# Avokadoen/zig_vulkan

Measured on AMD Instinct MI355X. Metric: Mrays/s at 1920x1080 on 512^3 brickmap (8^3 bricks, primary + shadow, 1 spp); achieved % of HBM roofline, higher is better.
Workload: dtype f32

## Files before the change

zig_vulkan_amd/csrc/vrt_trace_kernels.h:

```cpp
#pragma once
#include <hip/hip_runtime.h>
#include "vrt_internal.h"
#include "vrt_kernels.h"
#include "vrt_math.h"

namespace vrt {

constexpr uint32_t MAT_LAMBERTIAN = 0, MAT_METAL = 1, MAT_DIELECTRIC = 2, MAT_NONE = 3;

struct Ray {
    f3 origin, direction;
    float internal_reflection;
    uint32_t ignore_type_material;
};

struct Hit {
    f3 point, normal;
    float t;
    uint32_t index;
};

template <bool COUNT>
struct Cnt {
    uint32_t rays = 0, status_loads = 0, bricks_entered = 0, voxel_steps = 0, hits = 0, grid_steps = 0;
// ... 714 lines not shown
}

constexpr float kBoxMissEps = 1.0f / 64.0f;
constexpr float kBoxMissReach = 2048.0f;
VRT_DI bool box_miss(const f3 &origin, const f3 &inv_dir, const int (&bounds)[6], const f3 &g_min, float g_scale) {
    float reach = 0.0f;
    auto slab = [&](int k, float o, float inv, float g, float &near, float &far) {
        const float lo = ((float)(-bounds[k]) - (1.0f + kBoxMissEps)) * g_scale + g;
        const float hi = ((float)bounds[k + 3] + (2.0f + kBoxMissEps)) * g_scale + g;
        const float a0 = lo - o, a1 = hi - o;
        const float t0 = a0 * inv, t1 = a1 * inv;
        near = __builtin_fminf(t0, t1);
        far = __builtin_fmaxf(t0, t1);
        reach = __builtin_fmaxf(reach, __builtin_fmaxf(__builtin_fmaxf(__builtin_fabsf(a0), __builtin_fabsf(a1)), __builtin_fabsf(o)));
    };
    float nx, fx, ny, fy, nz, fz;
    slab(0, origin.x, inv_dir.x, g_min.x, nx, fx);
    slab(1, origin.y, inv_dir.y, g_min.y, ny, fy);
    slab(2, origin.z, inv_dir.z, g_min.z, nz, fz);
    const float tn = __builtin_fmaxf(__builtin_fmaxf(__builtin_fmaxf(nx, ny), nz), 0.0f);
    const float tf = __builtin_fminf(__builtin_fminf(fx, fy), fz);
    const float inv_max = __builtin_fmaxf(__builtin_fmaxf(__builtin_fabsf(inv_dir.x), __builtin_fabsf(inv_dir.y)), __builtin_fabsf(inv_dir.z));
    return tf < tn && reach <= kBoxMissReach * g_scale && inv_max < __builtin_inff();
}

struct BrickConsts {
    BrickArgs a;
    uint32_t occupancy_words;
    uint32_t start_is_slot;
    uint32_t scale_pow2;
    float inv_voxel_scale;
};
template <typename T>
VRT_DI T opaque_uniform(T v) {
    asm volatile("" : "+s"(v));
    return v;
}
template <typename T>
VRT_DI const __attribute__((address_space(1))) T *global_ptr(const T *ptr) {
    return (const __attribute__((address_space(1))) T *)ptr;
}
VRT_DI uint32_t scalar_load_u32(const uint32_t *ptr) {
    uint32_t v;
    asm volatile("s_load_dword %0, %1, 0x0\n\ts_waitcnt lgkmcnt(0)" : "=s"(v) : "s"(ptr));
    return v;
}
typedef __attribute__((ext_vector_type(8))) uint32_t u32x8;
typedef __attribute__((ext_vector_type(16))) uint32_t u32x16;
typedef __attribute__((ext_vector_type(2))) uint32_t u32x2;
VRT_DI unsigned long long kernarg_address() { return (unsigned long long)__builtin_amdgcn_kernarg_segment_ptr(); }
struct DerivedPtrs {
    const int *cell_bounds;
    const uint32_t *start_is_slot;
    uint32_t skip_to_box;
};
VRT_DI TileArgs kernarg_tile_args(DerivedPtrs &dp) {
    u32x16 v;
    u32x2 b, f;
    asm volatile("s_load_dwordx16 %0, %4, %5\n\ts_load_dwordx2 %1, %4, %6\n\ts_load_dwordx2 %2, %4, %7\n\ts_load_dword %3, %4, %8\n\ts_waitcnt lgkmcnt(0)"
                 : "=&s"(v), "=&s"(b), "=&s"(f), "=&s"(dp.skip_to_box)
                 : "s"(kernarg_address()), "n"(offsetof(TraceParams, tile_args)), "n"(offsetof(TraceParams, grid_extra) + offsetof(GridExtra, cell_bounds)),
                   "n"(offsetof(TraceParams, grid_extra) + offsetof(GridExtra, start_is_slot)), "n"(offsetof(TraceParams, grid_extra) + offsetof(GridExtra, skip_to_box)));
    dp.cell_bounds = (const int *)__builtin_bit_cast(unsigned long long, b);
    dp.start_is_slot = (const uint32_t *)__builtin_bit_cast(unsigned long long, f);
    return __builtin_bit_cast(TileArgs, v);
}

struct DerivedWords {
    int bounds[6];
    uint32_t start_is_slot;
};
struct EarlyBox {
    DerivedWords dw;
    float g_min[3], g_scale;
    bool test;
};
VRT_DI vrt_camera_device kernarg_camera_box(uint32_t frame, const DerivedPtrs &dp, EarlyBox &eb) {
    struct Parts { u32x16 a; u32x8 b; } v;
    u32x4 lo, gm;
    u32x2 hi;
    uint32_t flag, sc;
    const unsigned long long ka = kernarg_address();
    const unsigned long long at = ka + offsetof(TraceParams, pcs) + (unsigned long long)frame * sizeof(PushConstants);
    const unsigned long long b = dp.cell_bounds ? (unsigned long long)dp.cell_bounds : ka, f = dp.start_is_slot ? (unsigned long long)dp.start_is_slot : ka;
    asm volatile("s_load_dwordx16 %0, %7, 0x0\n\ts_load_dwordx8 %1, %7, 0x40\n\ts_load_dwordx4 %2, %8, 0x0\n\ts_load_dwordx2 %3, %8, 0x10\n\t"
                 "s_load_dword %4, %9, 0x0\n\ts_load_dwordx4 %5, %10, %11\n\ts_load_dword %6, %10, %12\n\ts_waitcnt lgkmcnt(0)"
                 : "=&s"(v.a), "=&s"(v.b), "=&s"(lo), "=&s"(hi), "=&s"(flag), "=&s"(gm), "=&s"(sc)
                 : "s"(at), "s"(b), "s"(f), "s"(ka), "n"(offsetof(TraceParams, grid) + offsetof(vrt_grid_state, min_point_base_t)),
                   "n"(offsetof(TraceParams, grid) + offsetof(vrt_grid_state, max_point_scale) + 12));
    eb.dw = DerivedWords{{(int)lo.x, (int)lo.y, (int)lo.z, (int)lo.w, (int)hi.x, (int)hi.y}, dp.start_is_slot ? flag : 0u};
    const uint32_t gx = gm.x, gy = gm.y, gz = gm.z;
    eb.g_min[0] = __builtin_bit_cast(float, gx), eb.g_min[1] = __builtin_bit_cast(float, gy), eb.g_min[2] = __builtin_bit_cast(float, gz);
    eb.g_scale = __builtin_bit_cast(float, sc);
    eb.test = dp.cell_bounds != nullptr && dp.skip_to_box != 0u;
    struct Padded { vrt_camera_device cam; uint32_t pad[8]; };
    static_assert(sizeof(Parts) == sizeof(Padded) && offsetof(Parts, b) == 64, "x16 | x8, padded to the alignment of the first");
    return __builtin_bit_cast(Padded, v).cam;
}
VRT_DI vrt_sun_device kernarg_sun(uint32_t frame) {
    u32x8 v;
    const unsigned long long at = kernarg_address() + offsetof(TraceParams, pcs) + (unsigned long long)frame * sizeof(PushConstants) + offsetof(PushConstants, sun);
    asm volatile("s_load_dwordx8 %0, %1, 0x0\n\ts_waitcnt lgkmcnt(0)" : "=&s"(v) : "s"(at));
    return __builtin_bit_cast(vrt_sun_device, v);
}
struct GridArgs {
    vrt_grid_state grid;
    uint32_t scale_pow2;
    float inv_grid_scale, inv_voxel_scale;
    uint32_t skip_to_box;
    const int *cell_bounds;
    uint32_t status_cells, status_words;
    const uint32_t *start_is_slot;
    uint32_t occupancy_words, count_box;
};
static_assert(sizeof(GridArgs) == sizeof(vrt_grid_state) + sizeof(GridExtra) && offsetof(GridArgs, cell_bounds) - 64 == offsetof(GridExtra, cell_bounds) &&
                  offsetof(GridArgs, start_is_slot) - 64 == offsetof(GridExtra, start_is_slot) && offsetof(GridArgs, count_box) - 64 == offsetof(GridExtra, count_box),
              "GridArgs = vrt_grid_state + GridExtra, field for field");
VRT_DI GridArgs kernarg_grid_args() {
    struct Parts { u32x16 grid; u32x8 a; u32x4 b; } v;
    asm volatile("s_load_dwordx16 %0, %3, 0x0\n\ts_load_dwordx8 %1, %3, %4\n\ts_load_dwordx4 %2, %3, %5\n\ts_waitcnt lgkmcnt(0)"
                 : "=&s"(v.grid), "=&s"(v.a), "=&s"(v.b)
                 : "s"(kernarg_address()), "n"(offsetof(TraceParams, grid_extra)), "n"(offsetof(TraceParams, grid_extra) + 32));
    static_assert(sizeof(Parts) == sizeof(GridArgs) + 16 && offsetof(Parts, a) == 64 && offsetof(Parts, b) == 96, "x16 | x8 | x4, padded to the alignment of the first");
    struct Padded { GridArgs g; uint32_t pad[4]; };
    return __builtin_bit_cast(Padded, v).g;
}
VRT_DI DerivedWords scalar_derived_words(const GridArgs &ga) {
    u32x4 lo;
    u32x2 hi;
    uint32_t flag;
    const unsigned long long ka = kernarg_address();
    const unsigned long long b = ga.cell_bounds ? (unsigned long long)ga.cell_bounds : ka, f = ga.start_is_slot ? (unsigned long long)ga.start_is_slot : ka;
    asm volatile("s_load_dwordx4 %0, %3, 0x0\n\ts_load_dwordx2 %1, %3, 0x10\n\ts_load_dword %2, %4, 0x0\n\ts_waitcnt lgkmcnt(0)"
                 : "=&s"(lo), "=&s"(hi), "=&s"(flag)
                 : "s"(b), "s"(f));
    return DerivedWords{{(int)lo.x, (int)lo.y, (int)lo.z, (int)lo.w, (int)hi.x, (int)hi.y}, ga.start_is_slot ? flag : 0u};
}
VRT_DI BrickConsts kernarg_brick_consts(const GridArgs &ga, uint32_t start_is_slot) {
    u32x16 v;
    asm volatile("s_load_dwordx16 %0, %1, %2\n\ts_waitcnt lgkmcnt(0)" : "=&s"(v) : "s"(kernarg_address()), "n"(offsetof(TraceParams, brick_args)));
    return BrickConsts{__builtin_bit_cast(BrickArgs, v), ga.occupancy_words, start_is_slot, ga.scale_pow2, ga.inv_voxel_scale};
}
VRT_DI int steps_left_fresh(int step, int pos, int dim, int zero_budget) {
    unsigned long long gt, lt;
    asm volatile("v_cmp_lt_i32_e64 %0, 0, %1" : "=s"(gt) : "v"(step));
    asm volatile("v_cmp_gt_i32_e64 %0, 0, %1" : "=s"(lt) : "v"(step));
    return __builtin_amdgcn_inverse_ballot_w64(gt) ? (int)((uint32_t)(dim - 1) - (uint32_t)pos) : (__builtin_amdgcn_inverse_ballot_w64(lt) ? pos : zero_budget);
}

template <int B, bool EAGER = true, bool BY_CELL = false, bool VOXEL = false, bool REJECT = false, bool CONSTS = false>
VRT_DI bool brick_walk_gfx950(const TraceParams &p, const BrickConsts &bc, const Ray &r, const RaySetup &s, float g_scale, uint32_t brick_index, f3 brick_min,
                              Hit &hit, int axis_in, int &hit_axis, uint32_t cell = 0u, uint32_t *hit_voxel = nullptr, uint32_t box = 0u) {
    constexpr bool kConsts = CONSTS;
    static_assert(!(CONSTS && BY_CELL), "the by-cell copy is the bounce kernel's");
    const float brick_voxel_scale = 1.0f / (float)B;
    const float voxel_scale = g_scale * brick_voxel_scale;
    const bool pow2 = kConsts ? opaque_uniform(bc.scale_pow2) != 0u : p.scale_pow2 != 0u;
    const f3 fposition = pow2 ? (ray_at(r, hit.t) - brick_min) * (kConsts ? bc.inv_voxel_scale : p.inv_voxel_scale) : (ray_at(r, hit.t) - brick_min) / splat3(voxel_scale);
    Walk w;
    w.side_dist = initial_side_dist(mk3((float)s.sx, (float)s.sy, (float)s.sz), fposition, s.ray_delta());
    const int px = f2i_clamp(__builtin_floorf(fposition.x));
    const int py = f2i_clamp(__builtin_floorf(fposition.y));
    const int pz = f2i_clamp(__builtin_floorf(fposition.z));
    constexpr int kZeroBudget = 3 * B + 8;
    w.rx = kConsts ? steps_left_fresh(s.sx, px, B, kZeroBudget) : steps_left(s.sx, px, B, kZeroBudget);
    w.ry = kConsts ? steps_left_fresh(s.sy, py, B, kZeroBudget) : steps_left(s.sy, py, B, kZeroBudget);
    w.rz = kConsts ? steps_left_fresh(s.sz, pz, B, kZeroBudget) : steps_left(s.sz, pz, B, kZeroBudget);
    w.t_value = 0;
    const float local_t_max = s.grid_t_max - hit.t;
    const bool by_cell = BY_CELL && p.cell_occupancy_lockstep != 0u;
    const uint32_t base = (by_cell ? cell : brick_index) * (uint32_t)(B * B * B);
    uint32_t bit_index = base + ((uint32_t)px + (uint32_t)B * ((uint32_t)pz + (uint32_t)B * (uint32_t)py));
    const uint32_t stride_x = (uint32_t)s.sx, stride_y = (uint32_t)(s.sy * (B * B)), stride_z = (uint32_t)(s.sz * B);
    bool more = more_init(px, py, pz, B) && (0.0f <= local_t_max);
    if constexpr (REJECT) {
        more = more && !brick_reject<B>(fposition, s.inv_dir, box);
        if (__builtin_amdgcn_ballot_w64(more) == 0ull) return false;
    }

    BrickArgs plain;
    if constexpr (!kConsts) plain.brick_occupancy = p.brick_occupancy, plain.brick_start_index = p.brick_start_index, plain.material_index = p.material_index, plain.materials = p.materials;
    const BrickArgs &a = kConsts ? bc.a : plain;
    const uint8_t *const occupancy = by_cell ? p.cell_occupancy : a.brick_occupancy;
    const unsigned long long occ_addr = (unsigned long long)occupancy;
    u32x4 rsrc;
    rsrc.x = (uint32_t)occ_addr;
    rsrc.y = (uint32_t)(occ_addr >> 32) | (4u << 16);
    rsrc.z = by_cell ? p.status_cells * (uint32_t)(B * B * B / 32) : (kConsts ? bc.occupancy_words : p.occupancy_words);
    rsrc.w = 0x00020000u;
    uint32_t word = global_ptr(reinterpret_cast<const uint32_t *>(occupancy))[more ? (bit_index >> 5) : 0u];
    uint32_t brick_material_index = 0u;
    bool start_is_slot;
    if constexpr (kConsts) start_is_slot = opaque_uniform(bc.start_is_slot) != 0u;
    else start_is_slot = p.start_is_slot != nullptr && __builtin_amdgcn_readfirstlane((int)*p.start_is_slot) != 0;
    if constexpr (EAGER) brick_material_index = start_is_slot ? brick_index * (uint32_t)(B * B * B) : (global_ptr(a.brick_start_index)[brick_index] & 0x7FFFFFFFu);
    GridWalkRegs g;
    g.alive = __builtin_amdgcn_ballot_w64(more);
    g.out_x = 0ull;
    g.out_y = 0ull;
    g.t_out = 0.0f;
    bool first = true;
    bool found = false;
    while (g.alive != 0ull) {
        uint32_t solid_bit;
        VRT_PROF_BEGIN(tp2);
        voxel_walk_gfx950(w, s.inv_dir, bit_index, solid_bit, stride_x, stride_y, stride_z, word, rsrc, g, voxel_scale, local_t_max);
        VRT_PROF_END(2, tp2);
        if (g.occ == 0ull) break;
        if (__builtin_amdgcn_inverse_ballot_w64(g.occ)) {
            VRT_PROF_BEGIN(tp4);
            const uint32_t voxel_index = solid_bit - base;
            if constexpr (!EAGER) brick_material_index = start_is_slot ? brick_index * (uint32_t)(B * B * B) : (global_ptr(a.brick_start_index)[brick_index] & 0x7FFFFFFFu);
            const uint32_t mi = global_ptr(a.material_index)[brick_material_index + voxel_index];
            const auto *m = global_ptr(kConsts ? opaque_uniform(a.materials) : a.materials) + mi;
            const uint32_t mtype = m->type;
            const float mdata = m->type_data;
            const bool ignore_brick = (mtype == r.ignore_type_material) && (r.internal_reflection == mdata);
            if (!ignore_brick) {
                const int a = (first && g.stub == 0u)
                                  ? axis_in
                                  : (__builtin_amdgcn_inverse_ballot_w64(g.in_x) ? 0 : (__builtin_amdgcn_inverse_ballot_w64(g.in_y) ? 1 : 2));
                hit.index = mi;
                const float t_offset = voxel_scale * 0.05f;
                hit.t += g.t_in * voxel_scale - t_offset;
                hit_axis = a;
                if constexpr (VOXEL) *hit_voxel = voxel_index;
                found = true;
            }
            VRT_PROF_END(4, tp4);
        }
        asm("s_andn2_b64 %0, %0, %1" : "+s"(g.alive) : "s"(__builtin_amdgcn_ballot_w64(found)) : "scc");
        first = false;
    }
    return found;
}

#ifndef VRT_BRICK_LOAD_AUX
#define VRT_BRICK_LOAD_AUX 0
#endif
VRT_DI void stage_brick_lds(const TraceParams &p, uint32_t occ_slot, bool by_cell, uint32_t wave_lds) {
    const uint32_t *src = reinterpret_cast<const uint32_t *>(by_cell ? p.cell_occupancy : p.brick_occupancy) + (size_t)occ_slot * 16u;
    typedef __attribute__((address_space(3))) void lds_void;
    typedef const __attribute__((address_space(1))) void glb_void;
    lds_void *dst = reinterpret_cast<lds_void *>((size_t)__builtin_amdgcn_readfirstlane(wave_lds));
#pragma unroll
    for (int c = 0; c < 4; c++)
        __builtin_amdgcn_global_load_lds((glb_void *)(src + 4 * c), (lds_void *)((__attribute__((address_space(3))) char *)dst + 1024 * c), 16, 0, VRT_BRICK_LOAD_AUX);
}
constexpr uint32_t kDeferredHit = 0x80000000u;
template <int B, bool LDS = false, bool PRESTAGED = false, bool DEFER = false>
VRT_DI bool brick_walk_park_gfx950(const TraceParams &p, const Ray &r, const RaySetup &s, float g_scale, uint32_t occ_slot, uint32_t cell, bool by_cell,
                                   bool start_is_slot, f3 brick_min, Hit &hit, int axis_in, int &hit_axis, uint32_t wave_lds = 0u) {
    static_assert(!LDS || B == 8, "the LDS layout is written for 64-byte bricks");
    const float brick_voxel_scale = 1.0f / (float)B;
    const float voxel_scale = g_scale * brick_voxel_scale;
    const f3 fposition = p.scale_pow2 ? (ray_at(r, hit.t) - brick_min) * p.inv_voxel_scale : (ray_at(r, hit.t) - brick_min) / splat3(voxel_scale);
    Walk w;
    w.side_dist = initial_side_dist(mk3((float)s.sx, (float)s.sy, (float)s.sz), fposition, s.ray_delta());
    const int px = f2i_clamp(__builtin_floorf(fposition.x));
    const int py = f2i_clamp(__builtin_floorf(fposition.y));
    const int pz = f2i_clamp(__builtin_floorf(fposition.z));
    constexpr int kZeroBudget = 3 * B + 8;
    w.rx = steps_left(s.sx, px, B, kZeroBudget);
    w.ry = steps_left(s.sy, py, B, kZeroBudget);
    w.rz = steps_left(s.sz, pz, B, kZeroBudget);
    w.t_value = 0;
    const float local_t_max = s.grid_t_max - hit.t;
    const uint32_t base = LDS ? 0u : occ_slot * (uint32_t)(B * B * B);
    uint32_t bit_index = base + ((uint32_t)px + (uint32_t)B * ((uint32_t)pz + (uint32_t)B * (uint32_t)py));
    const uint32_t stride_x = (uint32_t)s.sx, stride_y = (uint32_t)(s.sy * (B * B)), stride_z = (uint32_t)(s.sz * B);
    const bool more = more_init(px, py, pz, B) && (0.0f <= local_t_max);

    const uint8_t *const occupancy = by_cell ? p.cell_occupancy : p.brick_occupancy;
    const unsigned long long occ_addr = (unsigned long long)occupancy;
    u32x4 rsrc;
    rsrc.x = (uint32_t)occ_addr;
    rsrc.y = (uint32_t)(occ_addr >> 32) | (4u << 16);
    rsrc.z = by_cell ? p.status_cells * (uint32_t)(B * B * B / 32) : p.occupancy_words;
// ... 118 lines not shown
}
#undef VRT_SKIP_MERGE_STEP
VRT_DI float &comp3(f3 &v, int i) { return i == 0 ? v.x : (i == 1 ? v.y : v.z); }
VRT_DI float comp3(const f3 &v, int i) { return i == 0 ? v.x : (i == 1 ? v.y : v.z); }
template <int A>
VRT_DI void skip_axis(Walk &w, const RaySetup &s, int need, float t, uint32_t &index, uint32_t stride_x, uint32_t stride_y, uint32_t stride_z, bool &more,
                      int &in_axis, float &t_in) {
    constexpr int B1 = (A + 1) % 3, B2 = (A + 2) % 3;
    int *const r[3] = {&w.rx, &w.ry, &w.rz};
    const uint32_t stride[3] = {stride_x, stride_y, stride_z};
    const float t_strict = next_below(t);
    const int n1 = skip_merge_gfx950(comp3(w.side_dist, B1), comp3(s.inv_dir, B1), *r[B1], B1 > A ? t : t_strict);
    const int n2 = skip_merge_gfx950(comp3(w.side_dist, B2), comp3(s.inv_dir, B2), *r[B2], B2 > A ? t : t_strict);
    comp3(w.side_dist, A) = t + comp3(s.ray_delta(), A);
    *r[A] -= need;
    *r[B1] -= n1;
    *r[B2] -= n2;
    index += (uint32_t)need * stride[A] + (uint32_t)n1 * stride[B1] + (uint32_t)n2 * stride[B2];
    more = (*r[A] | *r[B1] | *r[B2]) >= 0;
    in_axis = A;
    t_in = t;
}
template <int A>
VRT_DI void skip_round(Walk &w, const RaySetup &s, int span, uint32_t &index, uint32_t stride_x, uint32_t stride_y, uint32_t stride_z, bool &more,
                       int &in_axis, float &t_in, bool &skipped) {
    const int step_a = A == 0 ? s.sx : (A == 1 ? s.sy : s.sz);
    const int r_a = A == 0 ? w.rx : (A == 1 ? w.ry : w.rz);
    const int need = step_a != 0 ? r_a - span : 0;
    const bool want = more && need > 0;
    if (__builtin_amdgcn_ballot_w64(want) == 0ull) return;
    if (want) {
        float t = comp3(w.side_dist, A);
        skip_add_gfx950(t, comp3(s.inv_dir, A), need - 1);
        skip_axis<A>(w, s, need, t, index, stride_x, stride_y, stride_z, more, in_axis, t_in);
        skipped = true;
    }
}
VRT_DI bool skip_to_box(Walk &w, const RaySetup &s, int span_x, int span_y, int span_z, uint32_t &index, uint32_t stride_x, uint32_t stride_y,
                        uint32_t stride_z, bool &more, int &in_axis, float &t_in) {
    bool skipped = false;
    skip_round<0>(w, s, span_x, index, stride_x, stride_y, stride_z, more, in_axis, t_in, skipped);
    skip_round<1>(w, s, span_y, index, stride_x, stride_y, stride_z, more, in_axis, t_in, skipped);
    skip_round<2>(w, s, span_z, index, stride_x, stride_y, stride_z, more, in_axis, t_in, skipped);
    return skipped;
}

#ifdef VRT_DEV_VARIANTS
#define VRT_DEV_SECTION 6
#include "vrt_trace_kernels_dev.h"
#undef VRT_DEV_SECTION
#endif
VRT_DI f3 opaque_uniform3(const float (&v)[3]) { return mk3(opaque_uniform(v[0]), opaque_uniform(v[1]), opaque_uniform(v[2])); }

template <int B, bool COUNT, int MODE, bool BATCH = false, bool SCALAR_ENTRY = false, bool VOXEL = false, bool REJECT = false, bool KARGS = false>
VRT_DI bool grid_hit(const TraceParams &p, const uint32_t *lds_filter, const Ray &r, Hit &hit, Cnt<COUNT> &c, int *voxel = nullptr,
                     const DerivedWords *early = nullptr, bool sits_out = false) {
    static_assert(!VOXEL || ((MODE == kStatusLinearAlways || MODE == kStatusLinearLds || MODE == kStatusBytes) && !COUNT && !BATCH),
                  "voxel coordinates come from the hand-written walk without batching");
    constexpr bool kHandWalk = (MODE == kStatusLinearAlways || MODE == kStatusLinearLds || MODE == kStatusBytes) && !COUNT;
    static_assert(!KARGS || (kHandWalk && !BATCH && MODE != kStatusLinearLds), "the batched arguments serve the one-sample kernels' walks");
    [[maybe_unused]] GridArgs ga;
    if constexpr (KARGS) ga = kernarg_grid_args();
#define VRT_GA(field) (KARGS ? ga.field : p.field)
    const float t_min = 0.00001f;
    const float t_max = __builtin_inff();
    VRT_COUNT(rays);
    VRT_PROF_BEGIN(tp3);
    RaySetup s;
    VRT_PROF_BEGIN(tp6);
    const bool slab_hit = grid_slab(VRT_GA(grid), r, t_min, t_max, s);
    VRT_PROF_END(6, tp6);
    if (!slab_hit || sits_out) return false;

    const f3 g_min = mk3(VRT_GA(grid.min_point_base_t)[0], VRT_GA(grid.min_point_base_t)[1], VRT_GA(grid.min_point_base_t)[2]);
    const float g_scale = VRT_GA(grid.max_point_scale)[3];
    const int dx = (int)VRT_GA(grid.dim_x), dy = (int)VRT_GA(grid.dim_y), dz = (int)VRT_GA(grid.dim_z);
    [[maybe_unused]] DerivedWords dw{};
    if constexpr (KARGS) dw = early ? *early : scalar_derived_words(ga);

    float global_t_value = s.grid_t_min + 0.0001f * (SCALAR_ENTRY ? opaque_uniform(g_scale) : g_scale);
    const f3 fposition = VRT_GA(scale_pow2) ? (ray_at(r, global_t_value) - g_min) * VRT_GA(inv_grid_scale) : (ray_at(r, global_t_value) - g_min) / splat3(g_scale);
    Walk w;
    w.side_dist = initial_side_dist(mk3((float)s.sx, (float)s.sy, (float)s.sz), fposition, s.ray_delta());
    const int px = f2i_clamp(__builtin_floorf(fposition.x));
    const int py = f2i_clamp(__builtin_floorf(fposition.y));
    const int pz = f2i_clamp(__builtin_floorf(fposition.z));
    const int zero_budget = dx + dy + dz + 8;
    int lox = 0, loy = 0, loz = 0, hix = dx - 1, hiy = dy - 1, hiz = dz - 1;
    if (!COUNT || VRT_GA(count_box)) {
        if (VRT_GA(cell_bounds)) {
            if constexpr (KARGS) {
                lox = -dw.bounds[0], loy = -dw.bounds[1], loz = -dw.bounds[2];
                hix = dw.bounds[3], hiy = dw.bounds[4], hiz = dw.bounds[5];
            } else {
                lox = -VRT_GA(cell_bounds)[0], loy = -VRT_GA(cell_bounds)[1], loz = -VRT_GA(cell_bounds)[2];
                hix = VRT_GA(cell_bounds)[3], hiy = VRT_GA(cell_bounds)[4], hiz = VRT_GA(cell_bounds)[5];
            }
        }
    }
    w.rx = steps_left_box(s.sx, px, lox, hix, zero_budget);
    w.ry = steps_left_box(s.sy, py, loy, hiy, zero_budget);
    w.rz = steps_left_box(s.sz, pz, loz, hiz, zero_budget);
    const int base_x = walk_base_box(s.sx, px, lox, hix), base_y = walk_base_box(s.sy, py, loy, hiy), base_z = walk_base_box(s.sz, pz, loz, hiz);
    w.t_value = 0;

    uint32_t word_index = ~0u;
    uint32_t word_bits = 0;
    uint32_t block_index = ~0u;
    uint2 block_bits = make_uint2(0u, 0u);
    int axis = 3;
    [[maybe_unused]] int hit_axis = 0;

    if (!(global_t_value <= t_max)) return false;
    uint32_t grid_index = (uint32_t)px + (uint32_t)dx * ((uint32_t)pz + (uint32_t)dz * (uint32_t)py);
    const uint32_t stride_x = (uint32_t)s.sx, stride_y = (uint32_t)s.sy * (uint32_t)dx * (uint32_t)dz, stride_z = (uint32_t)s.sz * (uint32_t)dx;

    int stop = 0;
    bool more = (unsigned)px < (unsigned)dx && (unsigned)py < (unsigned)dy && (unsigned)pz < (unsigned)dz && (w.rx | w.ry | w.rz) >= 0;
    [[maybe_unused]] bool skipped = false;
    [[maybe_unused]] float skip_t = 0.0f;
    if ((!COUNT || VRT_GA(count_box)) && VRT_GA(cell_bounds) && VRT_GA(skip_to_box)) {
        VRT_PROF_BEGIN(tp5);
        skipped = skip_to_box(w, s, (int)((uint32_t)hix - (uint32_t)lox), (int)((uint32_t)hiy - (uint32_t)loy), (int)((uint32_t)hiz - (uint32_t)loz), grid_index,
                              stride_x, stride_y, stride_z, more, axis, skip_t);
        w.t_value = skip_t;
        VRT_PROF_END(5, tp5);
    }

    [[maybe_unused]] BrickConsts bc{};
    if constexpr (KARGS) bc = kernarg_brick_consts(ga, dw.start_is_slot);

// ... 14 lines not shown
                const uint32_t wi = grid_index >> 5;
                if (wi != word_index) {
                    word_index = wi;
                    c.status_loads++;
                }
            }
            return status_bit(p.brick_status[grid_index >> 5], grid_index);
        } else if constexpr (MODE == kStatusLinear || MODE == kStatusLinearWide) {
            const uint32_t wi = grid_index >> 5;
            if (wi != word_index) {
                word_bits = p.brick_status[wi];
                word_index = wi;
                VRT_COUNT(status_loads);
            }
            return (word_bits >> (grid_index & 31u)) & 1u;
        } else {
            if constexpr (COUNT) {
                const uint32_t wi = grid_index >> 5;
                if (wi != word_index) {
                    word_index = wi;
                    c.status_loads++;
                }
            }
            const int cx = base_x - s.sx * w.rx, cy = base_y - s.sy * w.ry, cz = base_z - s.sz * w.rz;
            const uint32_t bi = (uint32_t)(cx >> 2) + p.nbx * ((uint32_t)(cz >> 2) + p.nbz * (uint32_t)(cy >> 2));
            if (bi != block_index) {
                block_index = bi;
                if constexpr (MODE == kStatusBlockedLds) {
                    const uint32_t fw = lds_filter[bi >> 5];
                    block_bits = ((fw >> (bi & 31u)) & 1u) ? p.status_blocks[bi] : make_uint2(0u, 0u);
                } else {
                    block_bits = p.status_blocks[bi];
                }
            }
            return bit64(block_bits, (uint32_t)((cx & 3) | ((cz & 3) << 2) | ((cy & 3) << 4)));
        }
    };
    auto enter_brick_at = [&](int rx, int ry, int rz, float t_cross, uint32_t cell, int &brick_axis) {
        const int cx = base_x - __mul24(s.sx, rx), cy = base_y - __mul24(s.sy, ry), cz = base_z - __mul24(s.sz, rz);
        const f3 brick_min = fma3(mk3((float)cx, (float)cy, (float)cz), splat3(g_scale), g_min);
        global_t_value = t_cross * g_scale + s.grid_t_min + 0.01f * g_scale;
        hit.t = global_t_value;
        const uint32_t brick_index = global_ptr(KARGS ? bc.a.brick_index : p.brick_index)[cell];
        [[maybe_unused]] uint32_t box = 0u;
        if constexpr (REJECT) {
            const uint32_t *const boxes = KARGS ? opaque_uniform(bc.a.cell_box) : p.cell_box;
            box = boxes ? global_ptr(boxes)[cell] : vrt::full_cell_box(B);
        }
        VRT_COUNT(bricks_entered);
        VRT_COUNT_WAVE(wave_brick_walks);
        bool found;
        if constexpr ((MODE == kStatusLinearAlways || MODE == kStatusLinearLds || MODE == kStatusBytes) && !COUNT) {
            [[maybe_unused]] uint32_t voxel_in_brick = 0u;
            found = brick_walk_gfx950<B, true, BATCH, VOXEL, REJECT, KARGS>(p, bc, r, s, g_scale, brick_index, brick_min, hit, brick_axis, hit_axis, cell, &voxel_in_brick, box);
            if constexpr (VOXEL) {
                if (found) {
                    voxel[0] = cx * B + (int)(voxel_in_brick % (uint32_t)B);
                    voxel[1] = cy * B + (int)(voxel_in_brick / (uint32_t)(B * B));
                    voxel[2] = cz * B + (int)((voxel_in_brick / (uint32_t)B) % (uint32_t)B);
                }
            }
        } else {
            found = brick_walk<B, COUNT, MODE == kStatusLinear || MODE == kStatusLinearLds || MODE == kStatusLinearAhead>(
                p, r, s, g_scale, brick_index, brick_min, hit, brick_axis, c);
        }
        stop = found ? -1 : ((global_t_value <= t_max) ? 0 : -2);
    };
    auto enter_brick = [&]() { enter_brick_at(w.rx, w.ry, w.rz, w.t_value, grid_index, axis); };
    auto finish_hit = [&]() {
        if constexpr ((MODE == kStatusLinearAlways || MODE == kStatusLinearLds || MODE == kStatusBytes) && !COUNT) {
            if (stop == -1) {
                const float t_offset = (g_scale * (1.0f / (float)B)) * 0.05f;
                hit.normal = axis_normal(s, hit_axis);
                hit.point = ray_at(r, hit.t) + hit.normal * t_offset;
            }
        }
    };

    if constexpr (BATCH && MODE == kStatusLinearAlways && !COUNT) {
        const unsigned long long status_addr = (unsigned long long)p.brick_status;
        u32x4 rsrc;
        rsrc.x = (uint32_t)status_addr;
        rsrc.y = (uint32_t)(status_addr >> 32) | (4u << 16);
        rsrc.z = p.status_words;
        rsrc.w = 0x00020000u;
        uint32_t word = p.brick_status[more ? (grid_index >> 5) : 0u];
        GridParkRegs g;
        g.alive = __builtin_amdgcn_ballot_w64(more);
        g.out_x = 0ull;
        g.out_y = 0ull;
        g.t_out = skip_t;
        g.code = (uint32_t)axis << 4;
        g.batch = p.brick_batch;
        VRT_PROF_END(3, tp3);
        while (g.alive != 0ull) {
            uint32_t cell;
            VRT_PROF_BEGIN(tp0);
            grid_walk_park_gfx950(w, s.inv_dir, grid_index, cell, stride_x, stride_y, stride_z, word, rsrc, g);
            VRT_PROF_END(0, tp0);
            if (g.parked == 0ull) break;
            const bool parked = __builtin_amdgcn_inverse_ballot_w64(g.parked);
            bool resume = false;
            VRT_PROF_BEGIN(tp1);
            if (parked) {
                int a = (int)(g.code & 3u);
                const uint32_t out = (g.code >> 2) & 3u;
                enter_brick_at(w.rx + (out == 0u ? 1 : 0), w.ry + (out == 1u ? 1 : 0), w.rz + (out == 2u ? 1 : 0), g.t_in, cell, a);
// ... 45 lines not shown
            int axis_here = axis;
            dda_step<true>(w, s.ray_delta(), g_scale, axis, grid_index, stride_x, stride_y, stride_z);
            const bool inside = min3i(w.rx, w.ry, w.rz) >= 0;
            word = inside ? p.brick_status[grid_index >> 5] : 0u;
            if (occupied) {
                const int a = axis;
                enter_brick_at(w.rx + (a == 0 ? 1 : 0), w.ry + (a == 1 ? 1 : 0), w.rz + (a == 2 ? 1 : 0), t_here,
                               grid_index - (a == 0 ? stride_x : (a == 1 ? stride_y : stride_z)), axis_here);
            }
            more = ((inside ? 0 : -1) | stop) >= 0;
        }
        return stop == -1;
    } else if constexpr ((MODE == kStatusLinearAlways || MODE == kStatusLinearLds || MODE == kStatusBytes) && !COUNT) {
        const unsigned long long status_addr = (MODE == kStatusBytes) ? (unsigned long long)(KARGS ? bc.a.status_bytes : p.status_bytes) : (unsigned long long)(KARGS ? bc.a.brick_status : p.brick_status);
        u32x4 rsrc;
        rsrc.x = (uint32_t)status_addr;
        rsrc.y = (uint32_t)(status_addr >> 32) | ((MODE == kStatusBytes) ? 0u : (4u << 16));
        rsrc.z = (MODE == kStatusBytes) ? VRT_GA(status_cells) : VRT_GA(status_words);
        rsrc.w = 0x00020000u;
        [[maybe_unused]] const uint32_t lds_mask = (0xFFFFFFFFu >> __builtin_clz(VRT_GA(status_words) * 4u - 1u)) & ~3u;
        uint32_t word;
        if constexpr (MODE == kStatusLinearLds) word = lds_word0(more ? (grid_index >> 5) : 0u);
        else if constexpr (MODE == kStatusBytes) word = global_ptr(KARGS ? bc.a.status_bytes : p.status_bytes)[more ? grid_index : 0u];
        else word = global_ptr(KARGS ? bc.a.brick_status : p.brick_status)[more ? (grid_index >> 5) : 0u];
        GridWalkRegs g;
        g.alive = __builtin_amdgcn_ballot_w64(more);
        g.out_x = __builtin_amdgcn_ballot_w64(skipped && axis == 0);
        g.out_y = __builtin_amdgcn_ballot_w64(skipped && axis == 1);
        g.t_out = skip_t;
        bool first = true;
        [[maybe_unused]] unsigned long long by_slab = 0ull;
        if constexpr (KARGS) by_slab = __builtin_amdgcn_ballot_w64(!skipped);
        VRT_PROF_END(3, tp3);
        while (g.alive != 0ull) {
            uint32_t cell;
            VRT_PROF_BEGIN(tp0);
            if constexpr (MODE == kStatusLinearLds) grid_walk_lds_gfx950(w, s.inv_dir, grid_index, cell, stride_x, stride_y, stride_z, word, lds_mask, g);
            else if constexpr (MODE == kStatusBytes) grid_walk_bytes_gfx950(w, s.inv_dir, grid_index, cell, stride_x, stride_y, stride_z, word, rsrc, g);
            else grid_walk_gfx950(w, s.inv_dir, grid_index, cell, stride_x, stride_y, stride_z, word, rsrc, g);
            VRT_PROF_END(0, tp0);
            if (g.occ == 0ull) break;
            if (__builtin_amdgcn_inverse_ballot_w64(g.occ)) {
                int a = (KARGS ? (__builtin_amdgcn_inverse_ballot_w64(by_slab) && g.stub == 0u) : (first && g.stub == 0u && !skipped)) ? 3
                                                : (__builtin_amdgcn_inverse_ballot_w64(g.in_x) ? 0 : (__builtin_amdgcn_inverse_ballot_w64(g.in_y) ? 1 : 2));
                const bool out_x = __builtin_amdgcn_inverse_ballot_w64(g.out_x), out_y = __builtin_amdgcn_inverse_ballot_w64(g.out_y);
                VRT_PROF_BEGIN(tp1);
                enter_brick_at(w.rx + (out_x ? 1 : 0), w.ry + (out_y ? 1 : 0), w.rz + ((out_x | out_y) ? 0 : 1), g.t_in, cell, a);
                VRT_PROF_END(1, tp1);
            }
            asm("s_andn2_b64 %0, %0, %1" : "+s"(g.alive) : "s"(__builtin_amdgcn_ballot_w64(stop != 0)) : "scc");
            first = false;
            if constexpr (KARGS) by_slab = 0ull;
        }
        finish_hit();
        return stop == -1;
    } else {
        while (more) {
            if (cell_occupied()) enter_brick();
            dda_step<true>(w, s.ray_delta(), g_scale, axis, grid_index, stride_x, stride_y, stride_z);
            more = (min3i(w.rx, w.ry, w.rz) | stop) >= 0;
        }
        return stop == -1;
    }
}
#undef VRT_GA

VRT_DI bool scatter_lambertian(const Hit &hit, Ray &scattered) {
    const f3 rv = rand_vec3_range(hit.point.x + hit.point.z, hit.point.y + hit.point.z, -0.4f, 0.4f);
    scattered = create_ray(hit.point, normalize3(hit.normal + rv));
    return true;
}
VRT_DI bool scatter_metal(float fuzz, const Ray &r_in, const Hit &hit, Ray &scattered) {
    const f3 reflected = reflect3(r_in.direction, hit.normal);
    const f3 rv = rand_vec3_range(hit.point.x + hit.point.z, hit.point.y + hit.point.z, -fuzz, fuzz);
    scattered = create_ray(hit.point, reflected + rv);
    return dot3(scattered.direction, hit.normal) > 0;
}
VRT_DI bool transmission_direction(float n1, float n2, f3 ray_dir, f3 normal, f3 &refrac_dir) {
    const float eta = n1 / n2;
    const float c1 = -dot3(ray_dir, normal);
    const float w = eta * c1;
    const float c2m = (w - eta) * (w + eta);
    if (c2m < -1.0f) return false;
    refrac_dir = fma3(splat3(eta), ray_dir, normal * (w - __builtin_sqrtf(1.0f + c2m)));
    return true;
}
VRT_DI bool scatter_dielectric(float ir, const Ray &r_in, const Hit &hit, Ray &scattered) {
    const f3 rv = rand_vec3_range(hit.point.x + hit.point.z, hit.point.y + hit.point.z, -0.05f, 0.05f);
    const f3 normal = normalize3(hit.normal + rv);
    f3 direction = mk3(0, 0, 0);
    const bool should_refract = transmission_direction(ir, r_in.internal_reflection, r_in.direction, normal, direction);
    if (should_refract && rand_3(hit.point) > 0.5f) {
        scattered = create_ray(hit.point, direction);
        scattered.ignore_type_material = MAT_DIELECTRIC;
        scattered.internal_reflection = ir;
    } else {
        direction = reflect3(r_in.direction, normal);
        scattered = create_ray(hit.point, direction);
    }
    return true;
}

template <int B, bool COUNT, int MODE, bool SCALAR_ENTRY = false, bool REJECT = false, bool KARGS = false>
VRT_DI f3 ray_color_single(const TraceParams &p, const PushConstants &pc, const uint32_t *lds_filter, const Ray &ray, Cnt<COUNT> &c,
                           const EarlyBox *eb = nullptr) {
    f3 color = mk3(0, 0, 0);
    int loop_count = 0;
    Hit hit;
    [[maybe_unused]] vrt_sun_device sun_batch;
    bool sun_enabled = false;
    f3 sun_color = mk3(0, 0, 0);
    if constexpr (!KARGS) sun_enabled = pc.sun.enabled > 0, sun_color = mk3(pc.sun.color[0], pc.sun.color[1], pc.sun.color[2]);
    bool primary_hit;
    if constexpr (KARGS) {
        const f3 inv = mk3(safe_inverse(ray.direction.x), safe_inverse(ray.direction.y), safe_inverse(ray.direction.z));
        const bool miss = eb->test && box_miss(ray.origin, inv, eb->dw.bounds, mk3(eb->g_min[0], eb->g_min[1], eb->g_min[2]), eb->g_scale);
        primary_hit = false;
        if (pc.cam.max_bounce > 0 && __builtin_amdgcn_ballot_w64(!miss) != 0ull) {
            primary_hit = grid_hit<B, COUNT, MODE, false, SCALAR_ENTRY, false, REJECT, KARGS>(p, lds_filter, ray, hit, c, nullptr, &eb->dw, miss);
        }
    } else {
        primary_hit = pc.cam.max_bounce > 0 && grid_hit<B, COUNT, MODE, false, SCALAR_ENTRY, false, REJECT, KARGS>(p, lds_filter, ray, hit, c);
    }
    if constexpr (KARGS) {
        sun_batch = kernarg_sun(blockIdx.y);
        sun_enabled = sun_batch.enabled > 0, sun_color = mk3(sun_batch.color[0], sun_batch.color[1], sun_batch.color[2]);
    }
    const vrt_sun_device &sun = KARGS ? sun_batch : pc.sun;
    if (primary_hit) {
        const uint32_t material = hit.index;
        bool lit = true;
        if (sun_enabled) {
            const f3 sun_position = mk3(sun.position[0], sun.position[1], sun.position[2]);
            const f3 rv = rand_vec3_range(ray.direction.x + ray.direction.z, ray.direction.y + ray.direction.z, -sun.radius,
                                          sun.radius);
            const Ray shadow_ray = create_ray(hit.point, (sun_position + rv) - hit.point);
            Hit shadow_hit;
            lit = !grid_hit<B, COUNT, MODE, false, SCALAR_ENTRY, false, REJECT, KARGS>(p, lds_filter, shadow_ray, shadow_hit, c);
        }
        const vrt_material *m = p.materials + material;
        const uint32_t mtype = m->type;
        const f3 attenuation = mk3(m->albedo_r, m->albedo_g, m->albedo_b);
        loop_count = (mtype <= MAT_DIELECTRIC) ? 1 : 0;
        if (sun_enabled) {
            if (lit) color = color + attenuation * sun_color;
        } else {
            color = color + attenuation;
        }
    }
    if (loop_count == 0) {
        const float t = 0.5f * (ray.direction.y + 1.0f);
        const f3 bg = fma3(splat3(1.0f - t), splat3(1.0f), mk3(0.5f, 0.7f, 1.0f) * t);
        color = color + bg * (sun_enabled ? sun_color : splat3(1.0f));
    }
    return color / (color + splat3(1.0f));
}

template <int B, bool COUNT, int MODE>
VRT_DI f3 ray_color(const TraceParams &p, const PushConstants &pc, const uint32_t *lds_filter, Ray current_ray, Cnt<COUNT> &c) {
    const bool sun_enabled = pc.sun.enabled > 0;
    const f3 sun_color = mk3(pc.sun.color[0], pc.sun.color[1], pc.sun.color[2]);
    const f3 sun_position = mk3(pc.sun.position[0], pc.sun.position[1], pc.sun.position[2]);
    const int max_bounce = pc.cam.max_bounce;
    Hit hit;
    hit.point = mk3(0, 0, 0);
    hit.normal = mk3(0, 0, 0);
    hit.t = 0;
    hit.index = 0;
    int loop_count = 0;
    f3 color = mk3(0, 0, 0);

    while (loop_count < max_bounce && grid_hit<B, COUNT, MODE, true, !COUNT>(p, lds_filter, current_ray, hit, c)) {
        loop_count += 1;
        Ray scattered = current_ray;
        bool result = false;
        const vrt_material *m = p.materials + hit.index;
        const uint32_t mtype = m->type;
        const f3 attenuation = mk3(m->albedo_r, m->albedo_g, m->albedo_b);
        const float mdata = m->type_data;
        switch (mtype) {
            case MAT_LAMBERTIAN: result = scatter_lambertian(hit, scattered); break;
            case MAT_METAL: result = scatter_metal(mdata, current_ray, hit, scattered); break;
            case MAT_DIELECTRIC: result = scatter_dielectric(mdata, current_ray, hit, scattered); break;
            default:
                loop_count -= 1;
                result = false;
                break;
        }
        if (sun_enabled) {
            const f3 rv = rand_vec3_range(current_ray.direction.x + current_ray.direction.z,
                                          current_ray.direction.y + current_ray.direction.z, -pc.sun.radius, pc.sun.radius);
// ... 240 lines not shown
```

Before: 39260.

## Skip per-voxel material lookups when materials are plain; any-hit shadow walks

```diff
diff --git a/zig_vulkan_amd/csrc/vrt_trace_kernels.h b/zig_vulkan_amd/csrc/vrt_trace_kernels.h
--- a/zig_vulkan_amd/csrc/vrt_trace_kernels.h
+++ b/zig_vulkan_amd/csrc/vrt_trace_kernels.h
@@ -790,24 +790,33 @@
 struct DerivedPtrs {
     const int *cell_bounds;
     const uint32_t *start_is_slot;
+    const uint32_t *materials_plain;
     uint32_t skip_to_box;
 };
 VRT_DI TileArgs kernarg_tile_args(DerivedPtrs &dp) {
     u32x16 v;
-    u32x2 b, f;
-    asm volatile("s_load_dwordx16 %0, %4, %5\n\ts_load_dwordx2 %1, %4, %6\n\ts_load_dwordx2 %2, %4, %7\n\ts_load_dword %3, %4, %8\n\ts_waitcnt lgkmcnt(0)"
-                 : "=&s"(v), "=&s"(b), "=&s"(f), "=&s"(dp.skip_to_box)
+    u32x2 b, f, m;
+    asm volatile("s_load_dwordx16 %0, %5, %6\n\ts_load_dwordx2 %1, %5, %7\n\ts_load_dwordx2 %2, %5, %8\n\ts_load_dword %3, %5, %9\n\ts_load_dwordx2 %4, %5, %10\n\t"
+                 "s_waitcnt lgkmcnt(0)"
+                 : "=&s"(v), "=&s"(b), "=&s"(f), "=&s"(dp.skip_to_box), "=&s"(m)
                  : "s"(kernarg_address()), "n"(offsetof(TraceParams, tile_args)), "n"(offsetof(TraceParams, grid_extra) + offsetof(GridExtra, cell_bounds)),
-                   "n"(offsetof(TraceParams, grid_extra) + offsetof(GridExtra, start_is_slot)), "n"(offsetof(TraceParams, grid_extra) + offsetof(GridExtra, skip_to_box)));
+                   "n"(offsetof(TraceParams, grid_extra) + offsetof(GridExtra, start_is_slot)), "n"(offsetof(TraceParams, grid_extra) + offsetof(GridExtra, skip_to_box)),
+                   "n"(offsetof(TraceParams, materials_plain)));
     dp.cell_bounds = (const int *)__builtin_bit_cast(unsigned long long, b);
     dp.start_is_slot = (const uint32_t *)__builtin_bit_cast(unsigned long long, f);
+    dp.materials_plain = (const uint32_t *)__builtin_bit_cast(unsigned long long, m);
     return __builtin_bit_cast(TileArgs, v);
 }
 
+constexpr uint32_t kFlagStartIsSlot = 1u, kFlagMaterialsPlain = 2u;
 struct DerivedWords {
     int bounds[6];
     uint32_t start_is_slot;
 };
+VRT_DI uint32_t derived_flags(const uint32_t *start_is_slot, uint32_t slot_word, const uint32_t *materials_plain, uint32_t plain_word) {
+    const uint32_t slot = start_is_slot ? slot_word : 0u, plain = materials_plain ? plain_word : 0u;
+    return (slot & 1u) | ((plain & 1u) << 1);
+}
 struct EarlyBox {
     DerivedWords dw;
     float g_min[3], g_scale;
@@ -817,16 +826,17 @@
     struct Parts { u32x16 a; u32x8 b; } v;
     u32x4 lo, gm;
     u32x2 hi;
-    uint32_t flag, sc;
+    uint32_t flag, sc, plain;
     const unsigned long long ka = kernarg_address();
     const unsigned long long at = ka + offsetof(TraceParams, pcs) + (unsigned long long)frame * sizeof(PushConstants);
     const unsigned long long b = dp.cell_bounds ? (unsigned long long)dp.cell_bounds : ka, f = dp.start_is_slot ? (unsigned long long)dp.start_is_slot : ka;
-    asm volatile("s_load_dwordx16 %0, %7, 0x0\n\ts_load_dwordx8 %1, %7, 0x40\n\ts_load_dwordx4 %2, %8, 0x0\n\ts_load_dwordx2 %3, %8, 0x10\n\t"
-                 "s_load_dword %4, %9, 0x0\n\ts_load_dwordx4 %5, %10, %11\n\ts_load_dword %6, %10, %12\n\ts_waitcnt lgkmcnt(0)"
-                 : "=&s"(v.a), "=&s"(v.b), "=&s"(lo), "=&s"(hi), "=&s"(flag), "=&s"(gm), "=&s"(sc)
+    const unsigned long long m = dp.materials_plain ? (unsigned long long)dp.materials_plain : ka;
+    asm volatile("s_load_dwordx16 %0, %8, 0x0\n\ts_load_dwordx8 %1, %8, 0x40\n\ts_load_dwordx4 %2, %9, 0x0\n\ts_load_dwordx2 %3, %9, 0x10\n\t"
+                 "s_load_dword %4, %10, 0x0\n\ts_load_dwordx4 %5, %11, %12\n\ts_load_dword %6, %11, %13\n\ts_load_dword %7, %14, 0x0\n\ts_waitcnt lgkmcnt(0)"
+                 : "=&s"(v.a), "=&s"(v.b), "=&s"(lo), "=&s"(hi), "=&s"(flag), "=&s"(gm), "=&s"(sc), "=&s"(plain)
                  : "s"(at), "s"(b), "s"(f), "s"(ka), "n"(offsetof(TraceParams, grid) + offsetof(vrt_grid_state, min_point_base_t)),
-                   "n"(offsetof(TraceParams, grid) + offsetof(vrt_grid_state, max_point_scale) + 12));
-    eb.dw = DerivedWords{{(int)lo.x, (int)lo.y, (int)lo.z, (int)lo.w, (int)hi.x, (int)hi.y}, dp.start_is_slot ? flag : 0u};
+                   "n"(offsetof(TraceParams, grid) + offsetof(vrt_grid_state, max_point_scale) + 12), "s"(m));
+    eb.dw = DerivedWords{{(int)lo.x, (int)lo.y, (int)lo.z, (int)lo.w, (int)hi.x, (int)hi.y}, derived_flags(dp.start_is_slot, flag, dp.materials_plain, plain)};
     const uint32_t gx = gm.x, gy = gm.y, gz = gm.z;
     eb.g_min[0] = __builtin_bit_cast(float, gx), eb.g_min[1] = __builtin_bit_cast(float, gy), eb.g_min[2] = __builtin_bit_cast(float, gz);
     eb.g_scale = __builtin_bit_cast(float, sc);
@@ -854,25 +864,28 @@
 static_assert(sizeof(GridArgs) == sizeof(vrt_grid_state) + sizeof(GridExtra) && offsetof(GridArgs, cell_bounds) - 64 == offsetof(GridExtra, cell_bounds) &&
                   offsetof(GridArgs, start_is_slot) - 64 == offsetof(GridExtra, start_is_slot) && offsetof(GridArgs, count_box) - 64 == offsetof(GridExtra, count_box),
               "GridArgs = vrt_grid_state + GridExtra, field for field");
-VRT_DI GridArgs kernarg_grid_args() {
+VRT_DI GridArgs kernarg_grid_args(const uint32_t *&materials_plain) {
     struct Parts { u32x16 grid; u32x8 a; u32x4 b; } v;
-    asm volatile("s_load_dwordx16 %0, %3, 0x0\n\ts_load_dwordx8 %1, %3, %4\n\ts_load_dwordx4 %2, %3, %5\n\ts_waitcnt lgkmcnt(0)"
-                 : "=&s"(v.grid), "=&s"(v.a), "=&s"(v.b)
-                 : "s"(kernarg_address()), "n"(offsetof(TraceParams, grid_extra)), "n"(offsetof(TraceParams, grid_extra) + 32));
+    u32x2 m;
+    asm volatile("s_load_dwordx16 %0, %4, 0x0\n\ts_load_dwordx8 %1, %4, %5\n\ts_load_dwordx4 %2, %4, %6\n\ts_load_dwordx2 %3, %4, %7\n\ts_waitcnt lgkmcnt(0)"
+                 : "=&s"(v.grid), "=&s"(v.a), "=&s"(v.b), "=&s"(m)
+                 : "s"(kernarg_address()), "n"(offsetof(TraceParams, grid_extra)), "n"(offsetof(TraceParams, grid_extra) + 32), "n"(offsetof(TraceParams, materials_plain)));
+    materials_plain = (const uint32_t *)__builtin_bit_cast(unsigned long long, m);
     static_assert(sizeof(Parts) == sizeof(GridArgs) + 16 && offsetof(Parts, a) == 64 && offsetof(Parts, b) == 96, "x16 | x8 | x4, padded to the alignment of the first");
     struct Padded { GridArgs g; uint32_t pad[4]; };
     return __builtin_bit_cast(Padded, v).g;
 }
-VRT_DI DerivedWords scalar_derived_words(const GridArgs &ga) {
+VRT_DI DerivedWords scalar_derived_words(const GridArgs &ga, const uint32_t *materials_plain) {
     u32x4 lo;
     u32x2 hi;
-    uint32_t flag;
+    uint32_t flag, plain;
     const unsigned long long ka = kernarg_address();
     const unsigned long long b = ga.cell_bounds ? (unsigned long long)ga.cell_bounds : ka, f = ga.start_is_slot ? (unsigned long long)ga.start_is_slot : ka;
-    asm volatile("s_load_dwordx4 %0, %3, 0x0\n\ts_load_dwordx2 %1, %3, 0x10\n\ts_load_dword %2, %4, 0x0\n\ts_waitcnt lgkmcnt(0)"
-                 : "=&s"(lo), "=&s"(hi), "=&s"(flag)
-                 : "s"(b), "s"(f));
-    return DerivedWords{{(int)lo.x, (int)lo.y, (int)lo.z, (int)lo.w, (int)hi.x, (int)hi.y}, ga.start_is_slot ? flag : 0u};
+    const unsigned long long m = materials_plain ? (unsigned long long)materials_plain : ka;
+    asm volatile("s_load_dwordx4 %0, %4, 0x0\n\ts_load_dwordx2 %1, %4, 0x10\n\ts_load_dword %2, %5, 0x0\n\ts_load_dword %3, %6, 0x0\n\ts_waitcnt lgkmcnt(0)"
+                 : "=&s"(lo), "=&s"(hi), "=&s"(flag), "=&s"(plain)
+                 : "s"(b), "s"(f), "s"(m));
+    return DerivedWords{{(int)lo.x, (int)lo.y, (int)lo.z, (int)lo.w, (int)hi.x, (int)hi.y}, derived_flags(ga.start_is_slot, flag, materials_plain, plain)};
 }
 VRT_DI BrickConsts kernarg_brick_consts(const GridArgs &ga, uint32_t start_is_slot) {
     u32x16 v;
@@ -886,11 +899,13 @@
     return __builtin_amdgcn_inverse_ballot_w64(gt) ? (int)((uint32_t)(dim - 1) - (uint32_t)pos) : (__builtin_amdgcn_inverse_ballot_w64(lt) ? pos : zero_budget);
 }
 
-template <int B, bool EAGER = true, bool BY_CELL = false, bool VOXEL = false, bool REJECT = false, bool CONSTS = false>
+constexpr int kPlainOff = 0, kPlainHit = 1, kPlainAnyHit = 2;
+template <int B, bool EAGER = true, bool BY_CELL = false, bool VOXEL = false, bool REJECT = false, bool CONSTS = false, int PLAIN = kPlainOff>
 VRT_DI bool brick_walk_gfx950(const TraceParams &p, const BrickConsts &bc, const Ray &r, const RaySetup &s, float g_scale, uint32_t brick_index, f3 brick_min,
                               Hit &hit, int axis_in, int &hit_axis, uint32_t cell = 0u, uint32_t *hit_voxel = nullptr, uint32_t box = 0u) {
     constexpr bool kConsts = CONSTS;
     static_assert(!(CONSTS && BY_CELL), "the by-cell copy is the bounce kernel's");
+    static_assert(PLAIN == kPlainOff || CONSTS, "the flags word is BrickConsts'");
     const float brick_voxel_scale = 1.0f / (float)B;
     const float voxel_scale = g_scale * brick_voxel_scale;
     const bool pow2 = kConsts ? opaque_uniform(bc.scale_pow2) != 0u : p.scale_pow2 != 0u;
@@ -911,6 +926,8 @@
     uint32_t bit_index = base + ((uint32_t)px + (uint32_t)B * ((uint32_t)pz + (uint32_t)B * (uint32_t)py));
     const uint32_t stride_x = (uint32_t)s.sx, stride_y = (uint32_t)(s.sy * (B * B)), stride_z = (uint32_t)(s.sz * B);
     bool more = more_init(px, py, pz, B) && (0.0f <= local_t_max);
+    [[maybe_unused]] uint32_t early_word = 0u;
+    if constexpr (kConsts && REJECT) early_word = global_ptr(reinterpret_cast<const uint32_t *>(bc.a.brick_occupancy))[more ? (bit_index >> 5) : 0u];
     if constexpr (REJECT) {
         more = more && !brick_reject<B>(fposition, s.inv_dir, box);
         if (__builtin_amdgcn_ballot_w64(more) == 0ull) return false;
@@ -926,10 +943,12 @@
     rsrc.y = (uint32_t)(occ_addr >> 32) | (4u << 16);
     rsrc.z = by_cell ? p.status_cells * (uint32_t)(B * B * B / 32) : (kConsts ? bc.occupancy_words : p.occupancy_words);
     rsrc.w = 0x00020000u;
-    uint32_t word = global_ptr(reinterpret_cast<const uint32_t *>(occupancy))[more ? (bit_index >> 5) : 0u];
+    uint32_t word;
+    if constexpr (kConsts && REJECT) word = early_word;
+    else word = global_ptr(reinterpret_cast<const uint32_t *>(occupancy))[more ? (bit_index >> 5) : 0u];
     uint32_t brick_material_index = 0u;
     bool start_is_slot;
-    if constexpr (kConsts) start_is_slot = opaque_uniform(bc.start_is_slot) != 0u;
+    if constexpr (kConsts) start_is_slot = (opaque_uniform(bc.start_is_slot) & kFlagStartIsSlot) != 0u;
     else start_is_slot = p.start_is_slot != nullptr && __builtin_amdgcn_readfirstlane((int)*p.start_is_slot) != 0;
     if constexpr (EAGER) brick_material_index = start_is_slot ? brick_index * (uint32_t)(B * B * B) : (global_ptr(a.brick_start_index)[brick_index] & 0x7FFFFFFFu);
     GridWalkRegs g;
@@ -949,19 +968,25 @@
             VRT_PROF_BEGIN(tp4);
             const uint32_t voxel_index = solid_bit - base;
             if constexpr (!EAGER) brick_material_index = start_is_slot ? brick_index * (uint32_t)(B * B * B) : (global_ptr(a.brick_start_index)[brick_index] & 0x7FFFFFFFu);
-            const uint32_t mi = global_ptr(a.material_index)[brick_material_index + voxel_index];
-            const auto *m = global_ptr(kConsts ? opaque_uniform(a.materials) : a.materials) + mi;
-            const uint32_t mtype = m->type;
-            const float mdata = m->type_data;
-            const bool ignore_brick = (mtype == r.ignore_type_material) && (r.internal_reflection == mdata);
+            uint32_t mi = brick_material_index + voxel_index;
+            bool ignore_brick = false;
+            if (PLAIN == kPlainOff || (opaque_uniform(bc.start_is_slot) & kFlagMaterialsPlain) == 0u) {
+                mi = global_ptr(a.material_index)[mi];
+                const auto *m = global_ptr(kConsts ? opaque_uniform(a.materials) : a.materials) + mi;
+                const uint32_t mtype = m->type;
+                const float mdata = m->type_data;
+                ignore_brick = (mtype == r.ignore_type_material) && (r.internal_reflection == mdata);
+            }
             if (!ignore_brick) {
-                const int a = (first && g.stub == 0u)
-                                  ? axis_in
-                                  : (__builtin_amdgcn_inverse_ballot_w64(g.in_x) ? 0 : (__builtin_amdgcn_inverse_ballot_w64(g.in_y) ? 1 : 2));
-                hit.index = mi;
-                const float t_offset = voxel_scale * 0.05f;
-                hit.t += g.t_in * voxel_scale - t_offset;
-                hit_axis = a;
+                if constexpr (PLAIN != kPlainAnyHit) {
+                    const int a = (first && g.stub == 0u)
+                                      ? axis_in
+                                      : (__builtin_amdgcn_inverse_ballot_w64(g.in_x) ? 0 : (__builtin_amdgcn_inverse_ballot_w64(g.in_y) ? 1 : 2));
+                    hit.index = mi;
+                    const float t_offset = voxel_scale * 0.05f;
+                    hit.t += g.t_in * voxel_scale - t_offset;
+                    hit_axis = a;
+                }
                 if constexpr (VOXEL) *hit_voxel = voxel_index;
                 found = true;
             }
@@ -1186,15 +1211,18 @@
 #endif
 VRT_DI f3 opaque_uniform3(const float (&v)[3]) { return mk3(opaque_uniform(v[0]), opaque_uniform(v[1]), opaque_uniform(v[2])); }
 
-template <int B, bool COUNT, int MODE, bool BATCH = false, bool SCALAR_ENTRY = false, bool VOXEL = false, bool REJECT = false, bool KARGS = false>
+template <int B, bool COUNT, int MODE, bool BATCH = false, bool SCALAR_ENTRY = false, bool VOXEL = false, bool REJECT = false, bool KARGS = false, bool ANY_HIT = false>
 VRT_DI bool grid_hit(const TraceParams &p, const uint32_t *lds_filter, const Ray &r, Hit &hit, Cnt<COUNT> &c, int *voxel = nullptr,
                      const DerivedWords *early = nullptr, bool sits_out = false) {
     static_assert(!VOXEL || ((MODE == kStatusLinearAlways || MODE == kStatusLinearLds || MODE == kStatusBytes) && !COUNT && !BATCH),
                   "voxel coordinates come from the hand-written walk without batching");
     constexpr bool kHandWalk = (MODE == kStatusLinearAlways || MODE == kStatusLinearLds || MODE == kStatusBytes) && !COUNT;
     static_assert(!KARGS || (kHandWalk && !BATCH && MODE != kStatusLinearLds), "the batched arguments serve the one-sample kernels' walks");
+    static_assert(!ANY_HIT || KARGS, "any-hit walks are the one-sample kernels' shadow rays");
+    constexpr int kPlain = !KARGS ? kPlainOff : (ANY_HIT ? kPlainAnyHit : kPlainHit);
     [[maybe_unused]] GridArgs ga;
-    if constexpr (KARGS) ga = kernarg_grid_args();
+    [[maybe_unused]] const uint32_t *plain_flag = nullptr;
+    if constexpr (KARGS) ga = kernarg_grid_args(plain_flag);
 #define VRT_GA(field) (KARGS ? ga.field : p.field)
     const float t_min = 0.00001f;
     const float t_max = __builtin_inff();
@@ -1210,7 +1238,7 @@
     const float g_scale = VRT_GA(grid.max_point_scale)[3];
     const int dx = (int)VRT_GA(grid.dim_x), dy = (int)VRT_GA(grid.dim_y), dz = (int)VRT_GA(grid.dim_z);
     [[maybe_unused]] DerivedWords dw{};
-    if constexpr (KARGS) dw = early ? *early : scalar_derived_words(ga);
+    if constexpr (KARGS) dw = early ? *early : scalar_derived_words(ga, plain_flag);
 
     float global_t_value = s.grid_t_min + 0.0001f * (SCALAR_ENTRY ? opaque_uniform(g_scale) : g_scale);
     const f3 fposition = VRT_GA(scale_pow2) ? (ray_at(r, global_t_value) - g_min) * VRT_GA(inv_grid_scale) : (ray_at(r, global_t_value) - g_min) / splat3(g_scale);
@@ -1331,7 +1359,7 @@
         bool found;
         if constexpr ((MODE == kStatusLinearAlways || MODE == kStatusLinearLds || MODE == kStatusBytes) && !COUNT) {
             [[maybe_unused]] uint32_t voxel_in_brick = 0u;
-            found = brick_walk_gfx950<B, true, BATCH, VOXEL, REJECT, KARGS>(p, bc, r, s, g_scale, brick_index, brick_min, hit, brick_axis, hit_axis, cell, &voxel_in_brick, box);
+            found = brick_walk_gfx950<B, true, BATCH, VOXEL, REJECT, KARGS, kPlain>(p, bc, r, s, g_scale, brick_index, brick_min, hit, brick_axis, hit_axis, cell, &voxel_in_brick, box);
             if constexpr (VOXEL) {
                 if (found) {
                     voxel[0] = cx * B + (int)(voxel_in_brick % (uint32_t)B);
@@ -1483,6 +1511,10 @@
             first = false;
             if constexpr (KARGS) by_slab = 0ull;
         }
+        if constexpr (ANY_HIT) return stop == -1;
+        if constexpr (kPlain == kPlainHit) {
+            if ((opaque_uniform(bc.start_is_slot) & kFlagMaterialsPlain) != 0u && stop == -1) hit.index = global_ptr(bc.a.material_index)[hit.index];
+        }
         finish_hit();
         return stop == -1;
     } else {
@@ -1567,7 +1599,7 @@
                                           sun.radius);
             const Ray shadow_ray = create_ray(hit.point, (sun_position + rv) - hit.point);
             Hit shadow_hit;
-            lit = !grid_hit<B, COUNT, MODE, false, SCALAR_ENTRY, false, REJECT, KARGS>(p, lds_filter, shadow_ray, shadow_hit, c);
+            lit = !grid_hit<B, COUNT, MODE, false, SCALAR_ENTRY, false, REJECT, KARGS, KARGS>(p, lds_filter, shadow_ray, shadow_hit, c);
         }
         const vrt_material *m = p.materials + material;
         const uint32_t mtype = m->type;
```

After: 40360 (median of 6 runs). +2.8%, better.
